# simon-ging/coot-videotext

Measured on AMD Instinct MI355X. Metric: clip-pairs/sec (COOT retrieval train step, whole job), higher is better.
Workload: dtype bf16; 1 GPU; ActivityNet-shaped paper config (anet_coot): 64 videos x 4 clips per GPU, Lc=Lv=80, Ls=16, Lp=64, Dv=2048, Dt=1536, d_model=384; global_batch_videos=64, parallelism=dp1, mode=train, launch=native, deterministic=True, batches=two different synthetic batches in turn

## Files before the change

### coot-videotext_amd/csrc/api.hip

```cpp
#include <stdarg.h>
#include <stdio.h>
#include <string.h>

#include <algorithm>
#include <mutex>
#include <string>
#include <unordered_map>
#include <vector>

#include "../../include/coot_hip.h"
#include "attention.h"
#include "common.h"
#include "fused.h"
#include "gemm.h"
#include "loss.h"
#include "pool.h"
#include "ref_f32.h"
#include "rowops.h"

namespace coot {

static thread_local char g_err[512] = "";
static thread_local hipStream_t g_glob_flush_stream = nullptr;
static thread_local hipEvent_t g_glob_flush_ev = nullptr;
// ... 568 lines not shown
using namespace coot;

extern "C" {

const char* coot_last_error(void) { return coot::g_err; }
int coot_version(void) { return COOT_ABI_VERSION; }
int coot_debug_dropout_scales(uint64_t seed, unsigned site, uint64_t idx0, int64_t n, float p, float* out_host) {
  COOT_REQUIRE(out_host && n >= 0 && p > 0.f, "debug_dropout_scales: bad arguments");
  const DropCfg d = mkdrop(1, p, seed, site);
  const unsigned key = drop_key(seed, site);
  for (int64_t i = 0; i < n; ++i) out_host[i] = drop_scale_key(key, idx0 + (uint64_t)i, d.thr, d.inv_keep);
  return 0;
}
int coot_debug_attn_dropout_scales(uint64_t seed, unsigned site, unsigned row32, int Lk, float p, float* out_host) {
  COOT_REQUIRE(out_host && Lk >= 0 && p > 0.f, "debug_attn_dropout_scales: bad arguments");
  const DropCfg d = mkdrop(1, p, seed, site);
  const unsigned key = drop_key(seed, site);
  for (int k = 0; k < Lk; ++k) out_host[k] = attn_drop_scale(key, row32, k, (unsigned)(Lk + 1) >> 1, d.thr, d.inv_keep);
  return 0;
}
int coot_debug_timestamps(void* dev_u64) { g_fz_tstamps = (unsigned long long*)dev_u64; return 0; }
extern "C" void coot_step_stamps_enable(int on);
extern "C" void coot_step_grad_write(int on);
extern "C" int coot_internal_stage_hits(void);
extern "C" int coot_internal_stream_counter(int which);
extern "C++" { namespace coot { int det_bypass_count(); } }
int coot_get_option(const char* name, int* value) {
  if (!value) { set_error("get_option: null result"); return -1; }
  if (!strcmp(name, "tn_dma")) { *value = get_tn_dma(); return 0; }
  if (!strcmp(name, "xcd_order")) { *value = get_xcd_order(); return 0; }
  if (!strcmp(name, "tn_mode")) { *value = get_tn_mode(); return 0; }
  if (!strcmp(name, "stage_hits")) { *value = coot_internal_stage_hits(); return 0; }
  if (!strcmp(name, "fused_attn_launches")) { *value = fused_attn_launches(); return 0; }
  if (!strcmp(name, "stream_overlap_tests")) { *value = coot_internal_stream_counter(0); return 0; }
  if (!strcmp(name, "stream_candidates_rejected")) { *value = coot_internal_stream_counter(1); return 0; }
  if (!strcmp(name, "stream_unresolved")) { *value = coot_internal_stream_counter(2); return 0; }
  if (!strcmp(name, "operand_f16")) { *value = COOT_OPERAND_IS_F16; return 0; }
  if (!strcmp(name, "det_bypasses")) { *value = det_bypass_count(); return 0; }
  set_error("get_option: unknown or write-only option %s", name);
  return -2;
}
int coot_set_option(const char* name, int value) {
  if (!strcmp(name, "tn_mode")) { set_tn_mode(value); return 0; }
  if (!strcmp(name, "step_stamps")) { coot_step_stamps_enable(value); return 0; }
  if (!strcmp(name, "fused")) { g_use_fused = value; return 0; }
  if (!strcmp(name, "glob_fused")) { g_use_glob_fused = value; return 0; }
  if (!strcmp(name, "glob_fused_bwd")) { g_use_glob_fused_bwd = value; return 0; }
  if (!strcmp(name, "packed")) { g_use_packed = value; return 0; }
  if (!strcmp(name, "fused_infc")) { g_use_fused_infc = value; return 0; }
  if (!strcmp(name, "fused_attn")) { set_fused_attn(value); return 0; }
  if (!strcmp(name, "tn_dma")) { set_tn_dma(value); return 0; }
  if (!strcmp(name, "pack_lazy")) { g_pack_lazy = value; return 0; }
  if (!strcmp(name, "pack_poison")) { g_pack_poison = value; return 0; }
  if (!strcmp(name, "grad_poison")) { g_grad_poison = value; return 0; }
  if (!strcmp(name, "tn_target_wgs")) { set_tn_target_wgs(value); return 0; }
  if (!strcmp(name, "xcd_order")) { set_xcd_order(value); return 0; }
  if (!strcmp(name, "grad_write")) { coot_step_grad_write(value); return 0; }
  if (!strcmp(name, "glob_flush_aux")) { g_glob_flush_aux = value; return 0; }
  if (!strcmp(name, "pool_handover")) { g_pool_handover_on = value; return 0; }
  if (!strcmp(name, "cl_col_split")) { set_cl_col_split(value); return 0; }
  if (!strcmp(name, "cl_small")) { set_cl_small(value); return 0; }
  if (!strcmp(name, "fz_debug")) { g_fz_debug = value; return 0; }
  if (!strcmp(name, "fused_min_rows")) { g_fused_min_rows = value; return 0; }
  set_error("unknown option %s", name);
  return -2;
}

int64_t coot_net_param_numel(const coot_net_config* cfg) {
  coot_net_config c; if (norm_cfg(cfg, &c)) return -1;
  NetLayout L; build_layout(c, L); return L.total;
}
int coot_net_param_count(const coot_net_config* cfg) {
  coot_net_config c; if (norm_cfg(cfg, &c)) return -1;
  NetLayout L; build_layout(c, L); return (int)L.entries.size();
}
int coot_net_param_info(const coot_net_config* cfg, int index, char* name, int name_len, int64_t* offset, int64_t shape[4], int* ndim) {
  coot_net_config c; RUN(norm_cfg(cfg, &c));
  NetLayout L; build_layout(c, L);
  COOT_REQUIRE(index >= 0 && index < (int)L.entries.size(), "param index %d out of range", index);
  const PEntry& e = L.entries[index];
// ... 155 lines not shown
  const coot_net_config* cfgs[1] = {cfg}; const float* Ps[1] = {P}; void* ws[1] = {wpack};
  return coot_nets_pack_weights(1, cfgs, Ps, ws, stream);
}

size_t coot_net_saved_bytes(const coot_net_config* cfg, int N, int Lseq, int N2, int L2) {
  coot_net_config c; if (norm_cfg(cfg, &c)) return 0;
  if (c.dtype == COOT_DTYPE_F32) {
    NetLayout L; build_layout(c, L);
    return ref_f32_workspace_bytes(ref_desc(c, L, N + N2), (long)N * Lseq + (long)N2 * L2);
  }
  Arena A(nullptr, 0); Saved S; layout_saved(c, N + N2, (long)N * Lseq + (long)N2 * L2, A, S); return A.off + 256;
}
size_t coot_net_scratch_bytes(const coot_net_config* cfg, int N, int Lseq, int N2, int L2) {
  coot_net_config c; if (norm_cfg(cfg, &c)) return 0;
  if (c.dtype == COOT_DTYPE_F32) {
    NetLayout L; build_layout(c, L);
    return ref_f32_scratch_bytes(ref_desc(c, L, N + N2), (long)N * Lseq + (long)N2 * L2);
  }
  Arena A(nullptr, 0); Scratch S; layout_scratch(c, N + N2, (long)N * Lseq + (long)N2 * L2, A, S); return A.off + 256;
}

static thread_local int g_grad_overwrite = 0;
int coot_net_grads_overwrite(int on) { g_grad_overwrite = on ? 1 : 0; return 0; }

struct ZeroRanges { float* p[64]; int n[64]; int poison[64]; int count; };
__global__ __launch_bounds__(256) void zero_ranges_kernel(ZeroRanges r) {
  float* p = r.p[blockIdx.x];
  const int n = r.n[blockIdx.x];
  const float v = r.poison[blockIdx.x] ? __uint_as_float(0x7FC00000u) : 0.f;
  for (int i = blockIdx.y * 256 + threadIdx.x; i < n; i += gridDim.y * 256) p[i] = v;
}
static void written_matrices(const coot_net_config& c, const NetLayout& L, std::vector<std::pair<int64_t, int64_t>>& mats) {
  const int64_t D = c.hidden_dim, F = c.ff_dim, Din = c.input_dim;
  if (c.use_input_fc) mats.push_back({L.in_w, D * Din});
  auto layer = [&](const LayerP& lp) { mats.push_back({lp.wqkv, 3 * D * D}); mats.push_back({lp.wo, D * D}); mats.push_back({lp.w1, F * D}); mats.push_back({lp.w2, D * F}); };
  for (const LayerP& lp : L.layers) layer(lp);
  for (const LayerP& lp : L.ctx) layer(lp);
  if (c.pooler == 0) { mats.push_back({L.pw1, D * (int64_t)c.pool_hidden}); mats.push_back({L.pw2, (int64_t)c.pool_hidden * (D / c.pool_heads)}); }
  std::sort(mats.begin(), mats.end());
}
int coot_debug_written_matrices(const coot_net_config* cfg, int64_t* offsets, int64_t* sizes, int max_ranges) {
  coot_net_config c; if (norm_cfg(cfg, &c)) return -1;
  NetLayout L; build_layout(c, L);
  std::vector<std::pair<int64_t, int64_t>> mats; written_matrices(c, L, mats);
  if ((int)mats.size() > max_ranges) return -1;
  for (size_t i = 0; i < mats.size(); ++i) { offsets[i] = mats[i].first; sizes[i] = mats[i].second; }
  return (int)mats.size();
}
int coot_nets_zero_grads(int nnets, const coot_net_config* const* cfgs, float* const* grads, int skip_matrices, coot_stream_t stream) {
  return coot_nets_zero_grads_ex(nnets, cfgs, grads, skip_matrices, nullptr, nullptr, 0, stream);
}
int coot_nets_zero_grads_ex(int nnets, const coot_net_config* const* cfgs, float* const* grads, int skip_matrices, float* const* extra,
                            const int64_t* extra_n, int n_extra, coot_stream_t stream) {
  hipStream_t st = (hipStream_t)stream;
  COOT_REQUIRE(nnets >= 1 && nnets <= 8 && cfgs && grads && (n_extra == 0 || (extra && extra_n)), "nets_zero_grads: bad arguments");
  ZeroRanges zr; zr.count = 0;
  auto flush = [&]() -> int {
    if (zr.count == 0) return 0;
    int big = 0;
    for (int i = 0; i < zr.count; ++i) if (zr.n[i] > big) big = zr.n[i];
    const int gy = big > (1 << 16) ? 64 : 2;
    hipLaunchKernelGGL(zero_ranges_kernel, dim3(zr.count, gy), dim3(256), 0, st, zr);
    COOT_CHECK_LAUNCH("zero_ranges");
    zr.count = 0;
    return 0;
  };
  auto add = [&](float* p, int64_t n, int poison) -> int {
    if (n <= 0) return 0;
    if (zr.count == 64) RUN(flush());
    zr.p[zr.count] = p; zr.n[zr.count] = (int)n; zr.poison[zr.count] = poison; ++zr.count;
    return 0;
  };
  for (int k = 0; k < nnets; ++k) {
    coot_net_config c; RUN(norm_cfg(cfgs[k], &c));
    NetLayout L; build_layout(c, L);
    if (!skip_matrices) { RUN(check_hip(hipMemsetAsync(grads[k], 0, (size_t)L.total * sizeof(float), st), "memset grads")); continue; }
    std::vector<std::pair<int64_t, int64_t>> mats; written_matrices(c, L, mats);
    int64_t pos = 0;
    for (const auto& m : mats) {
      COOT_REQUIRE(m.first >= pos && m.first + m.second <= L.total, "nets_zero_grads: parameter layout");
      RUN(add(grads[k] + pos, m.first - pos, 0));
      if (g_grad_poison) RUN(add(grads[k] + m.first, m.second, 1));
      pos = m.first + m.second;
    }
    RUN(add(grads[k] + pos, L.total - pos, 0));
  }
  for (int e = 0; e < n_extra; ++e)
    for (int64_t o = 0; o < extra_n[e]; o += (1 << 30)) RUN(add(extra[e] + o, extra_n[e] - o < (1 << 30) ? extra_n[e] - o : (1 << 30), 0));
  return flush();
}

struct InputStage { bf16_t* xhat = nullptr; int* pos = nullptr; int mode = 0; };
thread_local InputStage g_input_stage;
void coot_internal_set_input_stage(void* xhat, void* pos, int mode) {
  g_input_stage.xhat = (bf16_t*)xhat; g_input_stage.pos = (int*)pos; g_input_stage.mode = mode;
}

int coot_net_fwd(const coot_net_config* cfg, const float* P, const void* wpack, const float* pe, const float* feats,
                 const int64_t* lengths, int N, int Lseq, const float* feats2, const int64_t* lengths2, int N2, int L2,
                 const float* hidden, float* pooled, float* per_token, void* saved,
                 size_t saved_bytes, void* scratch, size_t scratch_bytes, int train, uint64_t seed, const uint64_t* seed_dev,
                 coot_stream_t stream, const coot_packed_seqs* packed) {
  hipStream_t st = (hipStream_t)stream;
  struct SeedScope { SeedScope(const uint64_t* p) { g_seed_dev = (const unsigned long long*)p; } ~SeedScope() { g_seed_dev = nullptr; } } seedscope(seed_dev);
  coot_net_config c; RUN(norm_cfg(cfg, &c));
  COOT_REQUIRE(P && wpack && pe && feats && lengths && pooled && saved, "net_fwd: null pointer");
  if (packed && packed->source != COOT_SOURCE_PADDED && N2 > 0 && !feats2) feats2 = feats;
  COOT_REQUIRE(!c.use_context || hidden, "net_fwd: context network needs hidden state (transformer_legacy.py:252)");
// ... 339 lines not shown
```

### coot-videotext_amd/csrc/api_step.hip

```cpp
#include <string.h>

#include "../../include/coot_hip.h"
#include "common.h"
#include "det.h"
#include "gemm.h"
#include "fused.h"
#include "pool.h"
#include "rowops.h"

#include <vector>
using namespace coot;

#define RUN(x) do { int _rc = (x); if (_rc) return _rc; } while (0)

namespace {

struct Bump {
  char* base; size_t cap; size_t off = 0; bool overflow = false;
  Bump(void* b, size_t c) : base((char*)b), cap(c) {}
  void* get(size_t bytes) {
    off = (off + 255) & ~(size_t)255;
    char* p = base ? base + off : nullptr;
    off += bytes;
    if (base && off > cap) overflow = true;
// ... 74 lines not shown
    made = true; return 0;
  }
  int hop(int slot, hipStream_t from, hipStream_t to) {
    if (from == to) return 0;
    RUN(record(slot, from));
    return wait(slot, to);
  }
  int record(int slot, hipStream_t from) {
    RUN(init());
    return check_hip(hipEventRecord(ev[slot], from), "eventRecord");
  }
  int wait(int slot, hipStream_t to) { return check_hip(hipStreamWaitEvent(to, ev[slot], 0), "streamWait"); }
};
thread_local Hops g_hops;
thread_local const uint64_t* g_step_seed_dev = nullptr;
thread_local int g_resh_wait_slot = -1;
thread_local void* g_glob_done[2] = {nullptr, nullptr};

constexpr long kEarlyMinTokens = 8192;
struct EarlyUpdate { bool on[2] = {false, false}; const coot_step_config* cfg = nullptr; const coot_step_buffers* b = nullptr; int64_t step = 0; bool repack = false; };
thread_local EarlyUpdate g_early;
int early_update_fire(int side, int gi, hipStream_t st);
int g_grad_write = 1;
int pack_nets(const coot_step_config& c, const coot_step_buffers& b, const int* nets, int count, void* stream) {
  const coot_net_config* cfgs[4]; const float* Ps[4]; void* ws[4];
  for (int k = 0; k < count; ++k) { cfgs[k] = &c.net[nets[k]]; Ps[k] = b.params[nets[k]]; ws[k] = b.wpack[nets[k]]; }
  return coot_nets_pack_weights(count, cfgs, Ps, ws, stream);
}

struct StepStamps {
  static constexpr int MAXN = 40;
  hipEvent_t ev[MAXN]; const char* label[MAXN]; int n = 0, made = 0; bool on = false;
  void begin() { n = 0; }
  void mark(const char* what, hipStream_t st) {
    if (!on || n >= MAXN) return;
    if (made <= n) { if (hipEventCreate(&ev[n]) != hipSuccess) return; made = n + 1; }
    if (hipEventRecord(ev[n], st) != hipSuccess) return;
    label[n++] = what;
  }
};
StepStamps g_stamps;

extern "C" void coot_internal_set_input_stage(void* xhat, void* pos, int mode);
extern "C" void coot_internal_set_glob_flush_stream(void* stream);
extern "C" void coot_internal_set_pool_pack(const long long* counts, int B, int Cmax, float* out, unsigned char* mask, long long* lens);
extern "C" int coot_internal_pool_handover_taken(void);
// ... 174 lines not shown
  glob_xcd_set(li == 0 ? 0 : 4, 4);
  const int rc_gf = coot_net_fwd(&c.net[gi], b.params[gi], b.wpack[gi], b.pe[gi], resh, item_num, d.B, Cmax, nullptr, nullptr, 0, 0,
                                 local_out , glob_out, nullptr, saved_g, sz_g, nullptr, 0, train, seed + 11 * gi,
                                 g_step_seed_dev, st, nullptr);
  glob_xcd_set(0, 8);
  RUN(rc_gf);
  g_stamps.mark(li == 0 ? "video: global forward done" : "text: global forward done", st);
  return 0;
}

int side_backward(const coot_step_config& c, const coot_step_buffers& b, int li, int gi, const float* ctx_feat, const int64_t* ctx_len,
                  int Lctx, const float* item_feat, const int64_t* item_len, int Litem, const int64_t* item_num, int Cmax,
                  const coot_step_dims& d, const float* local_out, const float* resh, float* d_local, const float* d_glob,
                  const float* d_resh, float* dhid, float* dfeat, void* saved_l, size_t sz_l, void* saved_g, size_t sz_g, void* scratch,
                  size_t sz_scratch, int train, uint64_t seed, hipStream_t st, const coot_packed_seqs* pk = nullptr) {
  const int D = c.net[0].hidden_dim;
  g_stamps.mark(li == 0 ? "video: backward starts" : "text: backward starts", st);
  const int side = li == 0 ? 0 : 1;
  const size_t sz_loc = align256(coot_net_scratch_bytes(&c.net[li], d.B, Lctx, d.Nc, Litem));
  const size_t sz_glob = coot_net_scratch_bytes(&c.net[gi], d.B, Cmax, 0, 0);
  COOT_REQUIRE(sz_loc + sz_glob <= sz_scratch, "step backward: scratch too small (%zu < %zu)", sz_scratch, sz_loc + sz_glob);
  glob_xcd_set(side == 0 ? 0 : 4, 4);
  if (g_early.on[side] && g_pipe.init() == 0) coot_internal_set_glob_flush_stream(g_pipe.stream);
  const int rc_g = coot_net_bwd(&c.net[gi], b.params[gi], b.wpack[gi], b.pe[gi], resh, item_num, d.B, Cmax, nullptr, nullptr, 0, 0, local_out, d_glob,
                                b.grads[gi], dhid, dfeat, saved_g, sz_g, (char*)scratch + sz_loc, sz_glob, train, seed + 11 * gi, g_step_seed_dev, st,
                                nullptr);
  glob_xcd_set(0, 8);
  coot_internal_set_glob_flush_stream(nullptr);
  RUN(rc_g);
  g_stamps.mark(li == 0 ? "video: global backward done" : "text: global backward done", st);
  if (g_glob_done[side]) {
    if (det_on()) RUN(det_flush_range(b.grads[gi], (size_t)coot_net_param_numel(&c.net[gi]) * sizeof(float), st));
    RUN(check_hip(hipEventRecord((hipEvent_t)g_glob_done[side], st), "eventRecord"));
  }
  if (g_early.on[side]) RUN(early_update_fire(side, gi, st));
  if (g_resh_wait_slot >= 0 && li == 0) RUN(g_hops.wait(g_resh_wait_slot, st));
  RUN(launch_pack_bwd_join(dfeat, d_resh, dhid, (const long long*)item_num, d.B, Cmax, D, d_local + (size_t)d.B * D, d_local, st));
  const int rc = coot_net_bwd(&c.net[li], b.params[li], b.wpack[li], b.pe[li], ctx_feat, ctx_len, d.B, Lctx, item_feat, item_len, d.Nc, Litem,
                              nullptr, d_local, b.grads[li], nullptr, nullptr, saved_l, sz_l, scratch, sz_loc, train, seed + 11 * li, g_step_seed_dev,
                              st, pk);
  RUN(rc);
  if (det_on()) {
    RUN(det_flush_range(b.grads[li], (size_t)coot_net_param_numel(&c.net[li]) * sizeof(float), st));
    RUN(det_flush_range(b.grads[gi], (size_t)coot_net_param_numel(&c.net[gi]) * sizeof(float), st));
  }
  g_stamps.mark(li == 0 ? "video: local backward done" : "text: local backward done", st);
  return 0;
}

__global__ void sample_idx_kernel(const long long* lens_a, const long long* lens_b, int B, unsigned long long seed, long long* idx,
                                  const unsigned long long* seed_dev = nullptr) {
  const int i = blockIdx.x * blockDim.x + threadIdx.x;
  if (i >= 2 * B) return;
  seed = eff_seed(seed, seed_dev);
  const long long len = i < B ? lens_a[i] : lens_b[i - B];
  const unsigned r = rng_u32(seed, 0xCCu, (unsigned long long)i);
  long long v = (long long)(((unsigned long long)r * (unsigned long long)len) >> 32);
  idx[i] = v < len ? v : len - 1;
}

struct OptK { int mode; float lr, b1, b2, eps, wd, a, b; };

__device__ __forceinline__ void opt_update(const OptK& k, float& p, float g, float& m, float& v, float d) {
  if (k.mode == 0) {
    const float gj = g + k.wd * d * p;
// ... 11 lines not shown
      p -= k.a * k.lr * m;
    }
  }
}

__device__ __forceinline__ void opt_update_range(const OptK& k, float* p, const float* g, float* m, float* v, const float* decay, long i, long n) {
  if (i + 3 < n) {
    f32x4_t pp = *reinterpret_cast<f32x4_t*>(p + i), gg = *reinterpret_cast<const f32x4_t*>(g + i);
    f32x4_t mm = *reinterpret_cast<f32x4_t*>(m + i), vv = *reinterpret_cast<f32x4_t*>(v + i);
    f32x4_t dd = decay ? *reinterpret_cast<const f32x4_t*>(decay + i) : f32x4_t{1.f, 1.f, 1.f, 1.f};
#pragma unroll
    for (int j = 0; j < 4; ++j) { float pj = pp[j], mj = mm[j], vj = vv[j]; opt_update(k, pj, gg[j], mj, vj, dd[j]); pp[j] = pj; mm[j] = mj; vv[j] = vj; }
    if (k.mode != 3) *reinterpret_cast<f32x4_t*>(p + i) = pp;
    *reinterpret_cast<f32x4_t*>(m + i) = mm; *reinterpret_cast<f32x4_t*>(v + i) = vv;
  } else {
    for (long e = i; e < n; ++e) opt_update(k, p[e], g[e], m[e], v[e], decay ? decay[e] : 1.f);
  }
}

__global__ __launch_bounds__(256) void adam_kernel(float* p, const float* g, float* m, float* v, const float* decay, long n, OptK k) {
  for (long i = ((long)blockIdx.x * 256 + threadIdx.x) * 4; i < n; i += (long)gridDim.x * 1024) opt_update_range(k, p, g, m, v, decay, i, n);
}

struct AdamSegs { float* p[4]; const float* g[4]; float* m[4]; float* v[4]; const float* decay[4]; const unsigned char* all1[4]; long n[4]; int blk0[5]; float* losses; };
__global__ __launch_bounds__(256) void adam4_kernel(AdamSegs sg, OptK k_arg, const OptK* k_dev) {
  const OptK k = k_dev ? *k_dev : k_arg;
  int s = 0;
#pragma unroll
  for (int t = 1; t < 4; ++t) if ((int)blockIdx.x >= sg.blk0[t]) s = t;
  if (sg.losses && blockIdx.x == 0 && threadIdx.x == 0) sg.losses[0] = sg.losses[1] + sg.losses[2];
  const long n = sg.n[s];
  const int blk = (int)blockIdx.x - sg.blk0[s];
  const long i = ((long)blk * 256 + threadIdx.x) * 4;
  if (i >= n) return;
  const float* decay = (sg.all1[s] && sg.all1[s][blk]) ? nullptr : sg.decay[s];
  opt_update_range(k, sg.p[s], sg.g[s], sg.m[s], sg.v[s], decay, i, n);
}

__host__ __device__ OptK opt_scalars(int optimizer, int radam_degentosgd, float lr, float beta1, float beta2, float eps, float wd, int64_t step) {
  OptK k; k.lr = lr; k.b1 = beta1; k.b2 = beta2; k.eps = eps; k.wd = wd; k.a = 0.f; k.b = 0.f;
  const double b1t = pow((double)beta1, (double)step), b2t = pow((double)beta2, (double)step);
  if (optimizer == 0) {
    k.mode = 0; k.a = (float)(1.0 / (1.0 - b1t)); k.b = (float)(1.0 / sqrt(1.0 - b2t));
  } else {
    const double nmax = 2.0 / (1.0 - (double)beta2) - 1.0;
    const double nsma = nmax - 2.0 * (double)step * b2t / (1.0 - b2t);
    if (nsma >= 5.0) {
      k.mode = 1;
      k.a = (float)(sqrt((1.0 - b2t) * (nsma - 4.0) / (nmax - 4.0) * (nsma - 2.0) / nsma * nmax / (nmax - 2.0)) / (1.0 - b1t));
    } else if (radam_degentosgd) {
      k.mode = 2; k.a = (float)(1.0 / (1.0 - b1t));
    } else {
      k.mode = 3;
    }
  }
  return k;
}

__global__ void loss_total_kernel(float* losses) { losses[0] = losses[1] + losses[2]; }

struct StepState { unsigned long long seed, step; float lr; int pad; OptK k; };
thread_local StepState* g_state_dev = nullptr;
__global__ void step_state_kernel(StepState* s, int optimizer, int degen, float b1, float b2, float eps, float wd, unsigned long long seed_inc) {
  s->step += 1; s->seed += seed_inc;
  s->k = opt_scalars(optimizer, degen, s->lr, b1, b2, eps, wd, (int64_t)s->step);
}

int adam_nets(const coot_step_config& cfg, const coot_step_buffers& b, const int* nets, int count, int64_t step, hipStream_t st,
              float* losses = nullptr) {
  AdamSegs sg;
  sg.losses = losses;
  int blk = 0;
  for (int k = 0; k < 4; ++k) {
    const int i = nets[k < count ? k : count - 1];
    const long n = k < count ? (long)coot_net_param_numel(&cfg.net[i]) : 0;
    sg.p[k] = b.params[i]; sg.g[k] = b.grads[i]; sg.m[k] = b.adam_m[i]; sg.v[k] = b.adam_v[i]; sg.decay[k] = b.decay_mask[i]; sg.n[k] = n;
    sg.all1[k] = b.decay_mask[i] ? b.decay_block_all[i] : nullptr;
    sg.blk0[k] = blk;
    blk += (int)((n / 4 + 255) / 256);
  }
  sg.blk0[4] = blk;
  const OptK k = opt_scalars(cfg.optimizer, cfg.radam_degentosgd, cfg.lr, cfg.beta1, cfg.beta2, cfg.eps, cfg.weight_decay, step);
  hipLaunchKernelGGL(adam4_kernel, dim3(blk), dim3(256), 0, st, sg, k, g_state_dev ? (const OptK*)&g_state_dev->k : (const OptK*)nullptr);
  COOT_CHECK_LAUNCH("adam4");
  return 0;
}

thread_local const int64_t* g_cc_idx_inject = nullptr;
int draw_cycle_indices(const coot_step_batch& x, const coot_step_dims& d, uint64_t seed, long long* idx, hipStream_t s) {
  if (g_cc_idx_inject)
    return check_hip(hipMemcpyAsync(idx, g_cc_idx_inject, 2 * (size_t)d.B * sizeof(long long), hipMemcpyDeviceToDevice, s), "cycle indices");
  hipLaunchKernelGGL(sample_idx_kernel, dim3((2 * d.B + 255) / 256), dim3(256), 0, s, (const long long*)x.clip_num, (const long long*)x.sent_num,
                     d.B, (unsigned long long)seed, idx, (const unsigned long long*)g_step_seed_dev);
  COOT_CHECK_LAUNCH("sample_idx");
  return 0;
}

int early_update_fire(int side, int gi, hipStream_t st) {
  RUN(g_pipe.init());
  RUN(g_hops.hop(11 + side, st, g_pipe.stream));
  const int nets[1] = {gi};
  RUN(adam_nets(*g_early.cfg, *g_early.b, nets, 1, g_early.step, g_pipe.stream));
  if (g_early.repack) RUN(pack_nets(*g_early.cfg, *g_early.b, nets, 1, g_pipe.stream));
  return g_hops.record(13 + side, g_pipe.stream);
}

}

extern "C" {

static int optimizer_step(int optimizer, int degen, float* params, const float* grads, float* m, float* v, const float* decay_mask, int64_t n,
                          float lr, float beta1, float beta2, float eps, float weight_decay, int64_t step, coot_stream_t stream) {
  COOT_REQUIRE(params && grads && m && v && step >= 1, "optimizer step: bad arguments");
  if (n <= 0) return 0;
  int blocks = (int)((n / 4 + 255) / 256);
  if (blocks > 2048) blocks = 2048;
  if (blocks < 1) blocks = 1;
  hipLaunchKernelGGL(adam_kernel, dim3(blocks), dim3(256), 0, (hipStream_t)stream, params, grads, m, v, decay_mask, (long)n,
                     opt_scalars(optimizer, degen, lr, beta1, beta2, eps, weight_decay, step));
  COOT_CHECK_LAUNCH("optimizer step");
  return 0;
}

int coot_adam_step(float* params, const float* grads, float* m, float* v, const float* decay_mask, int64_t n, float lr, float beta1,
                   float beta2, float eps, float weight_decay, int64_t step, coot_stream_t stream) {
// ... 169 lines not shown
  if (cc) {
    RUN(draw_cycle_indices(*x, *d, seed, W.idx, st));
    RUN(coot_cyclecons_fwd_bwd(W.resh_v, W.resh_t, x->clip_num, x->sent_num, (const int64_t*)W.idx, (const int64_t*)(W.idx + d->B), d->B,
                               d->Cmax_clip, d->Cmax_sent, D, cfg->cc_weight, 1.0f / (float)d->B, losses + 2, nullptr, nullptr, W.d_resh_v,
                               W.d_resh_t, side_t));
    g_stamps.mark("text: cycle-consistency done", st);
  }
  RUN(coot_contrastive_fwd_bwd_part(&cfg->contr, d->B, d->Nc, 2 * D, D, W.glob_v, W.glob_t, W.local_v + (size_t)d->B * D,
                                    W.local_t + (size_t)d->B * D, W.local_v, W.local_t, losses + 1, W.d_glob_v, W.d_glob_t,
                                    W.d_local_v + (size_t)d->B * D, W.d_local_t + (size_t)d->B * D, W.d_local_v, W.d_local_t, W.loss_scratch,
                                    W.sz_loss, COOT_CONTRASTIVE_LOCAL, side_t));
  g_stamps.mark("text: local contrastive terms done", st);
  RUN(g_hops.record(7, st));
  RUN(g_hops.wait(2, sv));
  g_stamps.mark("video: text forward joined", sv);
  RUN(coot_contrastive_fwd_bwd_part(&cfg->contr, d->B, d->Nc, 2 * D, D, W.glob_v, W.glob_t, W.local_v + (size_t)d->B * D,
                                    W.local_t + (size_t)d->B * D, W.local_v, W.local_t, losses + 1, W.d_glob_v, W.d_glob_t,
                                    W.d_local_v + (size_t)d->B * D, W.d_local_t + (size_t)d->B * D, W.d_local_v, W.d_local_t, W.loss_scratch,
                                    W.sz_loss, COOT_CONTRASTIVE_GLOBAL, side_v));
  g_stamps.mark("video: contrastive done", sv);
  RUN(g_hops.hop(3, sv, st));
  const int vnets[2] = {0, 1}, tnets[2] = {2, 3};
  g_resh_wait_slot = 7;
  const bool early = optimize && !det_on() && !g_state_dev;
  const bool early_v = early && (long)d->B * d->Lv + (long)d->Nc * d->Lc >= kEarlyMinTokens;
  const bool early_t = early && (long)d->B * d->Lp + (long)d->Nc * d->Ls >= kEarlyMinTokens;
  struct EarlyScope { ~EarlyScope() { g_early = EarlyUpdate{}; } } early_scope;
  g_early.on[0] = early_v; g_early.on[1] = early_t; g_early.cfg = cfg; g_early.b = b; g_early.step = step; g_early.repack = repack;
  (void)coot_net_grads_overwrite(g_grad_write);
  if (piped) coot_internal_set_input_stage(SL.xv, SL.pv, 0);
  const int rc_v = side_backward(*cfg, *b, 0, 1, x->vid_feat, x->vid_len, d->Lv, x->clip_feat, x->clip_len, d->Lc, x->clip_num, d->Cmax_clip, *d,
                                 W.local_v, W.resh_v, W.d_local_v, W.d_glob_v, cc ? W.d_resh_v : nullptr, W.dhid_v, W.dfeat_v, W.saved_lv, W.sz_lv,
                                 W.saved_gv, W.sz_gv, W.scratch_v, W.sz_sv, train, seed, sv, &pk.v);
  g_resh_wait_slot = -1;
  if (rc_v) (void)coot_net_grads_overwrite(0);
  RUN(rc_v);
  if (det_on()) RUN(det_flush_range(losses, 3 * sizeof(float), sv));
  if (optimize) RUN(adam_nets(*cfg, *b, vnets, early_v ? 1 : 2, step, sv, losses));
  else {
    hipLaunchKernelGGL(loss_total_kernel, dim3(1), dim3(1), 0, sv, losses);
    COOT_CHECK_LAUNCH("loss_total");
  }
  if (repack) RUN(pack_nets(*cfg, *b, vnets, early_v ? 1 : 2, side_v));
  if (early_v) RUN(g_hops.wait(13, sv));
  g_stamps.mark("video: updated", sv);
  if (piped) coot_internal_set_input_stage(SL.xt, SL.pt, 0);
  const int rc_t = side_backward(*cfg, *b, 2, 3, x->par_feat, x->par_len, d->Lp, x->sent_feat, x->sent_len, d->Ls, x->sent_num, d->Cmax_sent, *d, W.local_t,
                                 W.resh_t, W.d_local_t, W.d_glob_t, cc ? W.d_resh_t : nullptr, W.dhid_t, W.dfeat_t, W.saved_lt, W.sz_lt, W.saved_gt, W.sz_gt,
                                 W.scratch_t, W.sz_st, train, seed + 1000, st, &pk.t);
  (void)coot_net_grads_overwrite(0);
  coot_internal_set_input_stage(nullptr, nullptr, 0);
  RUN(rc_t);
  if (optimize) RUN(adam_nets(*cfg, *b, tnets, early_t ? 1 : 2, step, st));
  if (repack) RUN(pack_nets(*cfg, *b, tnets, early_t ? 1 : 2, side_t));
  if (early_t) RUN(g_hops.wait(14, st));
  g_stamps.mark("text: updated", st);
  RUN(g_hops.hop(4, sv, sm));
  if ((do_optimizer & COOT_STEP_DEFER_TEXT_JOIN) == 0) RUN(g_hops.hop(5, st, sm));
  g_stamps.mark("step done", sm);
  return 0;
}

void coot_step_stamps_enable(int on) { g_stamps.on = on != 0; }
int coot_internal_stage_hits(void) { return g_pipe.hits; }
size_t coot_step_device_state_bytes(void) { return sizeof(StepState); }
int coot_step_set_device_state(void* state) {
  g_state_dev = (StepState*)state;
  g_step_seed_dev = state ? (const uint64_t*)&g_state_dev->seed : nullptr;
  return 0;
}
int coot_step_set_cycle_indices(const int64_t* idx) { g_cc_idx_inject = idx; return 0; }
size_t coot_step_input_stage_bytes(const coot_step_config* cfg, const coot_step_dims* dims) {
  if (!cfg || !dims) return 0;
  return stage_layout(*cfg, *dims, nullptr).bytes;
}
int coot_step_set_input_stages(void* stage0, void* stage1, size_t bytes_each) {
// ... 50 lines not shown
  COOT_REQUIRE(out && n_others >= 0 && n_others <= 8 && (others || n_others == 0), "stream_create_concurrent: arguments");
  hipStream_t must[8];
  for (int i = 0; i < n_others; ++i) must[i] = (hipStream_t)others[i];
  hipStream_t s = nullptr;
  const hipStream_t nice[1] = {g_pipe.stream};
  RUN(g_streams.create(must, n_others, nice, g_pipe.stream ? 1 : 0, priority, &s, concurrent));
  g_streams.live.push_back(s);
  *out = (coot_stream_t)s;
  return 0;
}
int coot_stream_destroy(coot_stream_t s) {
  for (size_t i = 0; i < g_streams.live.size(); ++i)
    if (g_streams.live[i] == (hipStream_t)s) {
      g_streams.live.erase(g_streams.live.begin() + i);
      RUN(check_hip(hipStreamSynchronize((hipStream_t)s), "streamSynchronize"));
      if (g_pipe.checked && (g_pipe.beside[0] == (hipStream_t)s || g_pipe.beside[1] == (hipStream_t)s)) g_pipe.checked = false;
      return check_hip(hipStreamDestroy((hipStream_t)s), "streamDestroy");
    }
  set_error("stream_destroy: not a stream of coot_stream_create_concurrent (of this thread)");
  return 1;
}
int coot_internal_stream_counter(int which) { return which == 0 ? g_streams.tests : (which == 1 ? g_streams.rejected : g_streams.unresolved); }
void coot_step_grad_write(int on) { g_grad_write = on ? 1 : 0; }

int coot_debug_step_stamps(char* buf, int buf_bytes) {
  if (!buf || buf_bytes <= 0) return 0;
  buf[0] = 0;
  if (g_stamps.n == 0) return 0;
  if (hipDeviceSynchronize() != hipSuccess) return -1;
  int off = 0;
  for (int i = 0; i < g_stamps.n; ++i) {
    float ms = 0.f;
    if (hipEventElapsedTime(&ms, g_stamps.ev[0], g_stamps.ev[i]) != hipSuccess) ms = -1.f;
    off += snprintf(buf + off, off < buf_bytes ? buf_bytes - off : 0, "%9.1f us  %s\n", ms * 1e3f, g_stamps.label[i]);
    if (off >= buf_bytes) break;
  }
  return g_stamps.n;
}

}
```

### coot-videotext_amd/csrc/det.h

```cpp
#pragma once
#include "common.h"

namespace coot {

struct DetRange { const char* base; size_t bytes; long long* shadow; };
struct DetTable { int n; DetRange r[8]; unsigned* bypass; };
constexpr double kDetScale = 1099511627776.0;
constexpr float kDetMaxAddend = 4194304.0f;

static __device__ DetTable g_det_dev = {0, {}, nullptr};

__device__ __forceinline__ void acc_add(float* p, float v) {
  const int n = g_det_dev.n;
  for (int i = 0; i < n; ++i) {
    const size_t off = (size_t)(reinterpret_cast<const char*>(p) - g_det_dev.r[i].base);
    if (off < g_det_dev.r[i].bytes) {
      if (!(fabsf(v) < kDetMaxAddend)) {
        atomicAdd(g_det_dev.bypass, 1u);
        break;
      }
      atomicAdd(reinterpret_cast<unsigned long long*>(g_det_dev.r[i].shadow + (off >> 2)), (unsigned long long)llrint((double)v * kDetScale));
      return;
    }
  }
  atomicAdd(p, v);
}

#define COOT_DET_DEFINE_SETTER(name)                                                                              \
  int det_set_table_##name(const DetTable& t) {                                                                   \
    return check_hip(hipMemcpyToSymbol(HIP_SYMBOL(g_det_dev), &t, sizeof(DetTable)), "det table (" #name ")");   \
  }

int det_set_table_fused(const DetTable& t);
int det_set_table_gemm(const DetTable& t);
int det_set_table_loss(const DetTable& t);
int det_set_table_pool(const DetTable& t);
int det_set_table_rowops(const DetTable& t);
int det_flush_range(const void* base, size_t bytes, hipStream_t st);
bool det_on();
int det_bypass_count();

}
```

### coot-videotext_amd/csrc/det.hip

```cpp
#include "det.h"

#include "../../include/coot_hip.h"

namespace coot {
namespace {
DetTable g_host_table = {0, {}, nullptr};

__global__ __launch_bounds__(256) void det_flush_kernel(float* p, long long* shadow, long n) {
  for (long i = (long)blockIdx.x * 256 + threadIdx.x; i < n; i += (long)gridDim.x * 256) {
    const long long v = shadow[i];
    if (v != 0) {
      shadow[i] = 0;
      p[i] += (float)((double)v * (1.0 / kDetScale));
    }
  }
}
}

bool det_on() { return g_host_table.n > 0; }

int det_bypass_count() {
  if (g_host_table.n <= 0 || !g_host_table.bypass) return -1;
  unsigned v = 0;
  if (check_hip(hipDeviceSynchronize(), "det bypass count") || check_hip(hipMemcpy(&v, g_host_table.bypass, 4, hipMemcpyDeviceToHost), "det bypass count")) return -1;
  return (int)(v > 0x7fffffffu ? 0x7fffffffu : v);
}

int det_flush_range(const void* base, size_t bytes, hipStream_t st) {
  const char* b0 = (const char*)base;
  for (int i = 0; i < g_host_table.n; ++i) {
    const DetRange& R = g_host_table.r[i];
    const char* lo = b0 > R.base ? b0 : R.base;
    const char* hi = (b0 + bytes) < (R.base + R.bytes) ? (b0 + bytes) : (R.base + R.bytes);
    if (lo >= hi) continue;
    const long n = (hi - lo) / 4, first = (lo - R.base) / 4;
    int blocks = (int)((n + 1023) / 1024);
    if (blocks > 1024) blocks = 1024;
    if (blocks < 1) blocks = 1;
    hipLaunchKernelGGL(det_flush_kernel, dim3(blocks), dim3(256), 0, st, (float*)const_cast<char*>(lo), R.shadow + first, n);
// ... 46 lines not shown
```

### coot-videotext_amd/csrc/gemm.hip

```cpp
#include "gemm.h"
#include "det.h"
#include <algorithm>
#include "rowops.h"

namespace coot {

constexpr int BN = 128;
constexpr int BK = 64;
constexpr int PITCH = BK + 16;
constexpr int CPITCH = BN + 4;

__device__ __forceinline__ u32x4_t load16_guard(const bf16_t* p, bool ok) {
  u32x4_t z = {0u, 0u, 0u, 0u};
  if (ok) z = *reinterpret_cast<const u32x4_t*>(p);
  return z;
}

__device__ __forceinline__ void unpack8(u32x4_t u, float* v) {
  v[0] = bflo(u[0]); v[1] = bfhi(u[0]); v[2] = bflo(u[1]); v[3] = bfhi(u[1]);
  v[4] = bflo(u[2]); v[5] = bfhi(u[2]); v[6] = bflo(u[3]); v[7] = bfhi(u[3]);
}
__device__ __forceinline__ u32x4_t pack8(const float* v) {
  return u32x4_t{pack2bf(v[0], v[1]), pack2bf(v[2], v[3]), pack2bf(v[4], v[5]), pack2bf(v[6], v[7])};
}
// ... 1261 lines not shown
  if (g_tn_collect && !g.ws) {
    if (g_tn_nitems == TN_MAX_ITEMS) { int rc = tn_batch_flush(stream); if (rc) return rc; }
    g_tn_items[g_tn_nitems++] = g;
    return 0;
  }
  if (g.overwrite) {
    COOT_REQUIRE(g.groups == 1 && g.ldc == g.No, "gemm_tn: overwrite needs a dense single-group C");
    int rc = launch_fill_f32(g.C, (long)g.Mo * g.No, 0.f, stream);
    if (rc) return rc;
    GemmTN g2 = g; g2.overwrite = 0;
    return launch_gemm_tn(g2, stream);
  }
  int splits = tn_splits(g.T, g.Mo, g.No, g.groups);
  int t_per_split = (g.T + splits - 1) / splits;
  t_per_split = (t_per_split + TN_BT - 1) / TN_BT * TN_BT;
  splits = (g.T + t_per_split - 1) / t_per_split;
  float* ws = nullptr;
  const size_t need = (size_t)splits * g.groups * g.Mo * g.No;
  if (g.ws && need <= g.ws_floats) ws = g.ws;
  else if (!g.ws && g_tn_ws && need <= g_tn_ws_floats) ws = g_tn_ws;
  dim3 grid((g.No + TN_BC - 1) / TN_BC, (g.Mo + TN_BC - 1) / TN_BC, g.groups * splits);
  const int direct = (splits == 1 && g.ldc % 4 == 0 && g.No % 4 == 0 && g.zC % 4 == 0) ? 1 : 0;
  if (direct) ws = nullptr;
  void* ts = timing_begin(TIMING_TN, 2.0 * g.T * g.Mo * g.No * g.groups, 0, stream);
  if (g_tn_mode == 0)
    hipLaunchKernelGGL(gemm_tn_kernel<0>, grid, dim3(256), 0, stream, g, t_per_split, splits, ws, direct);
  else
    hipLaunchKernelGGL(gemm_tn_kernel<1>, grid, dim3(256), 0, stream, g, t_per_split, splits, ws, direct);
  COOT_CHECK_LAUNCH("gemm_tn");
  if (ws) {
    const long total4 = (long)g.Mo * g.No * g.groups / 4;
    int blocks = (int)((total4 + 255) / 256);
    if (blocks > 1024) blocks = 1024;
    hipLaunchKernelGGL(gemm_tn_reduce_kernel, dim3(blocks), dim3(256), 0, stream, g, splits, ws);
    COOT_CHECK_LAUNCH("gemm_tn_reduce");
  }
  timing_end(ts, stream);
  return 0;
}

}

namespace coot {
COOT_DET_DEFINE_SETTER(gemm)
}
```

Baseline: 207,700 clip-pairs/s.

## Fold deterministic shadow flush into Adam and restrict flush to accumulated gradient segments

In deterministic mode the whole gradient arena was flushed from its fixed-point shadow after each backward pass, and this blocked the early per-net optimizer update. The new code flushes only the gradient ranges that are actually accumulated atomically, and it folds that flush (plus the losses) into the Adam kernel itself. This re-enables early updates when deterministic mode is on. The cost is more per-block segment checks inside the Adam kernel and bookkeeping to detect split-K GEMMs that accumulate atomically.

```diff
diff --git a/coot-videotext_amd/csrc/api.hip b/coot-videotext_amd/csrc/api.hip
--- a/coot-videotext_amd/csrc/api.hip
+++ b/coot-videotext_amd/csrc/api.hip
@@ -614,6 +614,8 @@
 int coot_debug_timestamps(void* dev_u64) { g_fz_tstamps = (unsigned long long*)dev_u64; return 0; }
 extern "C" void coot_step_stamps_enable(int on);
 extern "C" void coot_step_grad_write(int on);
+extern "C" void coot_step_det_seg_flush(int on);
+extern "C" int coot_step_det_seg_flush_get(void);
 extern "C" int coot_internal_stage_hits(void);
 extern "C" int coot_internal_stream_counter(int which);
 extern "C++" { namespace coot { int det_bypass_count(); } }
@@ -628,6 +630,7 @@
   if (!strcmp(name, "stream_candidates_rejected")) { *value = coot_internal_stream_counter(1); return 0; }
   if (!strcmp(name, "stream_unresolved")) { *value = coot_internal_stream_counter(2); return 0; }
   if (!strcmp(name, "operand_f16")) { *value = COOT_OPERAND_IS_F16; return 0; }
+  if (!strcmp(name, "det_seg_flush")) { *value = coot_step_det_seg_flush_get(); return 0; }
   if (!strcmp(name, "det_bypasses")) { *value = det_bypass_count(); return 0; }
   set_error("get_option: unknown or write-only option %s", name);
   return -2;
@@ -648,6 +651,7 @@
   if (!strcmp(name, "tn_target_wgs")) { set_tn_target_wgs(value); return 0; }
   if (!strcmp(name, "xcd_order")) { set_xcd_order(value); return 0; }
   if (!strcmp(name, "grad_write")) { coot_step_grad_write(value); return 0; }
+  if (!strcmp(name, "det_seg_flush")) { coot_step_det_seg_flush(value); return 0; }
   if (!strcmp(name, "glob_flush_aux")) { g_glob_flush_aux = value; return 0; }
   if (!strcmp(name, "pool_handover")) { g_pool_handover_on = value; return 0; }
   if (!strcmp(name, "cl_col_split")) { set_cl_col_split(value); return 0; }
@@ -849,6 +853,7 @@
 
 static thread_local int g_grad_overwrite = 0;
 int coot_net_grads_overwrite(int on) { g_grad_overwrite = on ? 1 : 0; return 0; }
+extern "C" int coot_internal_grads_overwrite(void) { return g_grad_overwrite; }
 
 struct ZeroRanges { float* p[64]; int n[64]; int poison[64]; int count; };
 __global__ __launch_bounds__(256) void zero_ranges_kernel(ZeroRanges r) {
@@ -865,6 +870,27 @@
   for (const LayerP& lp : L.ctx) layer(lp);
   if (c.pooler == 0) { mats.push_back({L.pw1, D * (int64_t)c.pool_hidden}); mats.push_back({L.pw2, (int64_t)c.pool_hidden * (D / c.pool_heads)}); }
   std::sort(mats.begin(), mats.end());
+}
+static int accumulated_ranges(const coot_net_config& c, const NetLayout& L, std::vector<std::pair<int64_t, int64_t>>& acc,
+                              std::vector<std::pair<int64_t, int64_t>>* mats_out = nullptr) {
+  std::vector<std::pair<int64_t, int64_t>> mats; written_matrices(c, L, mats);
+  int64_t pos = 0;
+  for (const auto& m : mats) {
+    COOT_REQUIRE(m.first >= pos && m.first + m.second <= L.total, "gradient arena: parameter layout");
+    if (m.first > pos) acc.push_back({pos, m.first - pos});
+    pos = m.first + m.second;
+  }
+  if (L.total > pos) acc.push_back({pos, L.total - pos});
+  if (mats_out) *mats_out = mats;
+  return 0;
+}
+extern "C" int coot_internal_grad_accum_ranges(const coot_net_config* cfg, int64_t* offsets, int64_t* sizes, int max_ranges) {
+  coot_net_config c; RUN(norm_cfg(cfg, &c));
+  NetLayout L; build_layout(c, L);
+  std::vector<std::pair<int64_t, int64_t>> acc; RUN(accumulated_ranges(c, L, acc));
+  COOT_REQUIRE((int)acc.size() <= max_ranges, "grad_accum_ranges: %d ranges (room for %d)", (int)acc.size(), max_ranges);
+  for (size_t i = 0; i < acc.size(); ++i) { offsets[i] = acc[i].first; sizes[i] = acc[i].second; }
+  return (int)acc.size();
 }
 int coot_debug_written_matrices(const coot_net_config* cfg, int64_t* offsets, int64_t* sizes, int max_ranges) {
   coot_net_config c; if (norm_cfg(cfg, &c)) return -1;
@@ -902,15 +928,10 @@
     coot_net_config c; RUN(norm_cfg(cfgs[k], &c));
     NetLayout L; build_layout(c, L);
     if (!skip_matrices) { RUN(check_hip(hipMemsetAsync(grads[k], 0, (size_t)L.total * sizeof(float), st), "memset grads")); continue; }
-    std::vector<std::pair<int64_t, int64_t>> mats; written_matrices(c, L, mats);
-    int64_t pos = 0;
-    for (const auto& m : mats) {
-      COOT_REQUIRE(m.first >= pos && m.first + m.second <= L.total, "nets_zero_grads: parameter layout");
-      RUN(add(grads[k] + pos, m.first - pos, 0));
-      if (g_grad_poison) RUN(add(grads[k] + m.first, m.second, 1));
-      pos = m.first + m.second;
-    }
-    RUN(add(grads[k] + pos, L.total - pos, 0));
+    std::vector<std::pair<int64_t, int64_t>> acc, mats; RUN(accumulated_ranges(c, L, acc, &mats));
+    for (const auto& a : acc) RUN(add(grads[k] + a.first, a.second, 0));
+    if (g_grad_poison)
+      for (const auto& m : mats) RUN(add(grads[k] + m.first, m.second, 1));
   }
   for (int e = 0; e < n_extra; ++e)
     for (int64_t o = 0; o < extra_n[e]; o += (1 << 30)) RUN(add(extra[e] + o, extra_n[e] - o < (1 << 30) ? extra_n[e] - o : (1 << 30), 0));
diff --git a/coot-videotext_amd/csrc/api_step.hip b/coot-videotext_amd/csrc/api_step.hip
--- a/coot-videotext_amd/csrc/api_step.hip
+++ b/coot-videotext_amd/csrc/api_step.hip
@@ -120,6 +120,26 @@
 thread_local EarlyUpdate g_early;
 int early_update_fire(int side, int gi, hipStream_t st);
 int g_grad_write = 1;
+
+extern "C" int coot_internal_grad_accum_ranges(const coot_net_config* cfg, int64_t* offsets, int64_t* sizes, int max_ranges);
+extern "C" int coot_internal_grads_overwrite(void);
+int g_det_seg = 1;
+struct DetPlan {
+  bool fold = false;
+  bool full[4] = {true, true, true, true};
+  float* losses = nullptr;
+};
+thread_local DetPlan g_det_plan;
+int det_arena_segs(const coot_step_config& c, const coot_step_buffers& b, int net, DetSegs& out, hipStream_t st) {
+  const long n = (long)coot_net_param_numel(&c.net[net]);
+  if (g_det_plan.full[net]) return det_segs_add(out, b.grads[net], n, st);
+  int64_t off[64], len[64];
+  const int k = coot_internal_grad_accum_ranges(&c.net[net], off, len, 64);
+  if (k < 0) return k;
+  for (int i = 0; i < k; ++i) RUN(det_segs_add(out, b.grads[net] + off[i], (long)len[i], st));
+  return 0;
+}
+void det_plan_arena(int net) { g_det_plan.full[net] = !coot_internal_grads_overwrite() || det_take_matrix_atomics(); }
 int pack_nets(const coot_step_config& c, const coot_step_buffers& b, const int* nets, int count, void* stream) {
   const coot_net_config* cfgs[4]; const float* Ps[4]; void* ws[4];
   for (int k = 0; k < count; ++k) { cfgs[k] = &c.net[nets[k]]; Ps[k] = b.params[nets[k]]; ws[k] = b.wpack[nets[k]]; }
@@ -340,25 +360,42 @@
   COOT_REQUIRE(sz_loc + sz_glob <= sz_scratch, "step backward: scratch too small (%zu < %zu)", sz_scratch, sz_loc + sz_glob);
   glob_xcd_set(side == 0 ? 0 : 4, 4);
   if (g_early.on[side] && g_pipe.init() == 0) coot_internal_set_glob_flush_stream(g_pipe.stream);
+  (void)det_take_matrix_atomics();
   const int rc_g = coot_net_bwd(&c.net[gi], b.params[gi], b.wpack[gi], b.pe[gi], resh, item_num, d.B, Cmax, nullptr, nullptr, 0, 0, local_out, d_glob,
                                 b.grads[gi], dhid, dfeat, saved_g, sz_g, (char*)scratch + sz_loc, sz_glob, train, seed + 11 * gi, g_step_seed_dev, st,
                                 nullptr);
   glob_xcd_set(0, 8);
   coot_internal_set_glob_flush_stream(nullptr);
   RUN(rc_g);
+  det_plan_arena(gi);
   g_stamps.mark(li == 0 ? "video: global backward done" : "text: global backward done", st);
+  const bool seg = det_on() && g_det_seg;
   if (g_glob_done[side]) {
-    if (det_on()) RUN(det_flush_range(b.grads[gi], (size_t)coot_net_param_numel(&c.net[gi]) * sizeof(float), st));
+    if (seg) {
+      DetSegs ds;
+      RUN(det_arena_segs(c, b, gi, ds, st));
+      RUN(det_flush_segs(ds, st));
+    } else if (det_on()) {
+      RUN(det_flush_range(b.grads[gi], (size_t)coot_net_param_numel(&c.net[gi]) * sizeof(float), st));
+    }
     RUN(check_hip(hipEventRecord((hipEvent_t)g_glob_done[side], st), "eventRecord"));
   }
   if (g_early.on[side]) RUN(early_update_fire(side, gi, st));
   if (g_resh_wait_slot >= 0 && li == 0) RUN(g_hops.wait(g_resh_wait_slot, st));
   RUN(launch_pack_bwd_join(dfeat, d_resh, dhid, (const long long*)item_num, d.B, Cmax, D, d_local + (size_t)d.B * D, d_local, st));
+  (void)det_take_matrix_atomics();
   const int rc = coot_net_bwd(&c.net[li], b.params[li], b.wpack[li], b.pe[li], ctx_feat, ctx_len, d.B, Lctx, item_feat, item_len, d.Nc, Litem,
                               nullptr, d_local, b.grads[li], nullptr, nullptr, saved_l, sz_l, scratch, sz_loc, train, seed + 11 * li, g_step_seed_dev,
                               st, pk);
   RUN(rc);
-  if (det_on()) {
+  det_plan_arena(li);
+  if (seg && !g_det_plan.fold) {
+    DetSegs ds;
+    RUN(det_arena_segs(c, b, li, ds, st));
+    if (!g_glob_done[side]) RUN(det_arena_segs(c, b, gi, ds, st));
+    if (side == 0 && g_det_plan.losses) RUN(det_segs_add(ds, g_det_plan.losses, 3, st));
+    RUN(det_flush_segs(ds, st));
+  } else if (det_on() && !seg) {
     RUN(det_flush_range(b.grads[li], (size_t)coot_net_param_numel(&c.net[li]) * sizeof(float), st));
     RUN(det_flush_range(b.grads[gi], (size_t)coot_net_param_numel(&c.net[gi]) * sizeof(float), st));
   }
@@ -416,17 +453,43 @@
   for (long i = ((long)blockIdx.x * 256 + threadIdx.x) * 4; i < n; i += (long)gridDim.x * 1024) opt_update_range(k, p, g, m, v, decay, i, n);
 }
 
-struct AdamSegs { float* p[4]; const float* g[4]; float* m[4]; float* v[4]; const float* decay[4]; const unsigned char* all1[4]; long n[4]; int blk0[5]; float* losses; };
+constexpr int kAdamFlushSegs = 64;
+struct AdamSegs {
+  float* p[4]; float* g[4]; float* m[4]; float* v[4]; const float* decay[4]; const unsigned char* all1[4]; long n[4]; int blk0[5]; float* losses;
+  long long* sh[4]; long long* loss_sh; int fseg0[5]; int flo[kAdamFlushSegs], fhi[kAdamFlushSegs];
+};
 __global__ __launch_bounds__(256) void adam4_kernel(AdamSegs sg, OptK k_arg, const OptK* k_dev) {
   const OptK k = k_dev ? *k_dev : k_arg;
   int s = 0;
 #pragma unroll
   for (int t = 1; t < 4; ++t) if ((int)blockIdx.x >= sg.blk0[t]) s = t;
-  if (sg.losses && blockIdx.x == 0 && threadIdx.x == 0) sg.losses[0] = sg.losses[1] + sg.losses[2];
+  if (sg.losses && blockIdx.x == 0 && threadIdx.x == 0) {
+    if (sg.loss_sh)
+      for (int w = 0; w < 3; ++w) {
+        const long long v = sg.loss_sh[w];
+        if (v != 0) { sg.loss_sh[w] = 0; sg.losses[w] = det_fold(sg.losses[w], v); }
+      }
+    sg.losses[0] = sg.losses[1] + sg.losses[2];
+  }
   const long n = sg.n[s];
   const int blk = (int)blockIdx.x - sg.blk0[s];
   const long i = ((long)blk * 256 + threadIdx.x) * 4;
   if (i >= n) return;
+  if (long long* sh = sg.sh[s]) {
+    const long b0 = (long)blk * 1024, b1 = b0 + 1024;
+    float* g = sg.g[s];
+    for (int q = sg.fseg0[s]; q < sg.fseg0[s + 1]; ++q) {
+      const long lo = sg.flo[q], hi = sg.fhi[q];
+      if (lo >= b1 || hi <= b0) continue;
+#pragma unroll
+      for (int j = 0; j < 4; ++j) {
+        const long e = i + j;
+        if (e < lo || e >= hi || e >= n) continue;
+        const long long v = sh[e];
+        if (v != 0) { sh[e] = 0; g[e] = det_fold(g[e], v); }
+      }
+    }
+  }
   const float* decay = (sg.all1[s] && sg.all1[s][blk]) ? nullptr : sg.decay[s];
   opt_update_range(k, sg.p[s], sg.g[s], sg.m[s], sg.v[s], decay, i, n);
 }
@@ -461,10 +524,17 @@
 }
 
 int adam_nets(const coot_step_config& cfg, const coot_step_buffers& b, const int* nets, int count, int64_t step, hipStream_t st,
-              float* losses = nullptr) {
+              float* losses = nullptr, bool flush = false) {
   AdamSegs sg;
   sg.losses = losses;
-  int blk = 0;
+  sg.loss_sh = nullptr;
+  flush = flush && det_on();
+  DetSegs spill;
+  if (flush && losses) {
+    const int where = det_locate(losses, 3 * sizeof(float), &sg.loss_sh);
+    if (where < 0) RUN(det_segs_add(spill, losses, 3, st));
+  }
+  int blk = 0, nseg = 0;
   for (int k = 0; k < 4; ++k) {
     const int i = nets[k < count ? k : count - 1];
     const long n = k < count ? (long)coot_net_param_numel(&cfg.net[i]) : 0;
@@ -472,8 +542,24 @@
     sg.all1[k] = b.decay_mask[i] ? b.decay_block_all[i] : nullptr;
     sg.blk0[k] = blk;
     blk += (int)((n / 4 + 255) / 256);
-  }
-  sg.blk0[4] = blk;
+    sg.sh[k] = nullptr; sg.fseg0[k] = nseg;
+    if (!flush || k >= count) continue;
+    DetSegs ds;
+    RUN(det_arena_segs(cfg, b, i, ds, st));
+    if (ds.n == 0) continue;
+    bool fits = nseg + ds.n <= kAdamFlushSegs && n <= (1L << 30);
+    for (int q = 0; q < ds.n && fits; ++q) fits = ds.s[q].shadow - (ds.s[q].p - b.grads[i]) == ds.s[0].shadow - (ds.s[0].p - b.grads[i]);
+    if (!fits) {
+      for (int q = 0; q < ds.n; ++q) RUN(det_segs_add(spill, ds.s[q].p, ds.s[q].n, st));
+      continue;
+    }
+    sg.sh[k] = ds.s[0].shadow - (ds.s[0].p - b.grads[i]);
+    for (int q = 0; q < ds.n; ++q) {
+      sg.flo[nseg] = (int)(ds.s[q].p - b.grads[i]); sg.fhi[nseg] = sg.flo[nseg] + ds.s[q].n; ++nseg;
+    }
+  }
+  sg.blk0[4] = blk; sg.fseg0[4] = nseg;
+  RUN(det_flush_segs(spill, st));
   const OptK k = opt_scalars(cfg.optimizer, cfg.radam_degentosgd, cfg.lr, cfg.beta1, cfg.beta2, cfg.eps, cfg.weight_decay, step);
   hipLaunchKernelGGL(adam4_kernel, dim3(blk), dim3(256), 0, st, sg, k, g_state_dev ? (const OptK*)&g_state_dev->k : (const OptK*)nullptr);
   COOT_CHECK_LAUNCH("adam4");
@@ -494,7 +580,7 @@
   RUN(g_pipe.init());
   RUN(g_hops.hop(11 + side, st, g_pipe.stream));
   const int nets[1] = {gi};
-  RUN(adam_nets(*g_early.cfg, *g_early.b, nets, 1, g_early.step, g_pipe.stream));
+  RUN(adam_nets(*g_early.cfg, *g_early.b, nets, 1, g_early.step, g_pipe.stream, nullptr, g_det_plan.fold));
   if (g_early.repack) RUN(pack_nets(*g_early.cfg, *g_early.b, nets, 1, g_pipe.stream));
   return g_hops.record(13 + side, g_pipe.stream);
 }
@@ -710,7 +796,9 @@
   RUN(g_hops.hop(3, sv, st));
   const int vnets[2] = {0, 1}, tnets[2] = {2, 3};
   g_resh_wait_slot = 7;
-  const bool early = optimize && !det_on() && !g_state_dev;
+  struct DetScope { ~DetScope() { g_det_plan = DetPlan{}; } } det_scope;
+  g_det_plan.fold = optimize && g_det_seg; g_det_plan.losses = losses;
+  const bool early = optimize && (!det_on() || g_det_seg) && !g_state_dev;
   const bool early_v = early && (long)d->B * d->Lv + (long)d->Nc * d->Lc >= kEarlyMinTokens;
   const bool early_t = early && (long)d->B * d->Lp + (long)d->Nc * d->Ls >= kEarlyMinTokens;
   struct EarlyScope { ~EarlyScope() { g_early = EarlyUpdate{}; } } early_scope;
@@ -723,8 +811,8 @@
   g_resh_wait_slot = -1;
   if (rc_v) (void)coot_net_grads_overwrite(0);
   RUN(rc_v);
-  if (det_on()) RUN(det_flush_range(losses, 3 * sizeof(float), sv));
-  if (optimize) RUN(adam_nets(*cfg, *b, vnets, early_v ? 1 : 2, step, sv, losses));
+  if (det_on() && !g_det_seg) RUN(det_flush_range(losses, 3 * sizeof(float), sv));
+  if (optimize) RUN(adam_nets(*cfg, *b, vnets, early_v ? 1 : 2, step, sv, losses, g_det_plan.fold));
   else {
     hipLaunchKernelGGL(loss_total_kernel, dim3(1), dim3(1), 0, sv, losses);
     COOT_CHECK_LAUNCH("loss_total");
@@ -739,7 +827,7 @@
   (void)coot_net_grads_overwrite(0);
   coot_internal_set_input_stage(nullptr, nullptr, 0);
   RUN(rc_t);
-  if (optimize) RUN(adam_nets(*cfg, *b, tnets, early_t ? 1 : 2, step, st));
+  if (optimize) RUN(adam_nets(*cfg, *b, tnets, early_t ? 1 : 2, step, st, nullptr, g_det_plan.fold));
   if (repack) RUN(pack_nets(*cfg, *b, tnets, early_t ? 1 : 2, side_t));
   if (early_t) RUN(g_hops.wait(14, st));
   g_stamps.mark("text: updated", st);
@@ -836,6 +924,8 @@
 }
 int coot_internal_stream_counter(int which) { return which == 0 ? g_streams.tests : (which == 1 ? g_streams.rejected : g_streams.unresolved); }
 void coot_step_grad_write(int on) { g_grad_write = on ? 1 : 0; }
+void coot_step_det_seg_flush(int on) { g_det_seg = on ? 1 : 0; }
+int coot_step_det_seg_flush_get(void) { return g_det_seg; }
 
 int coot_debug_step_stamps(char* buf, int buf_bytes) {
   if (!buf || buf_bytes <= 0) return 0;
diff --git a/coot-videotext_amd/csrc/det.h b/coot-videotext_amd/csrc/det.h
--- a/coot-videotext_amd/csrc/det.h
+++ b/coot-videotext_amd/csrc/det.h
@@ -37,6 +37,17 @@
 int det_set_table_pool(const DetTable& t);
 int det_set_table_rowops(const DetTable& t);
 int det_flush_range(const void* base, size_t bytes, hipStream_t st);
+
+__device__ __forceinline__ float det_fold(float w, long long v) { return __fadd_rn(w, (float)((double)v * (1.0 / kDetScale))); }
+
+int det_locate(const void* base, size_t bytes, long long** shadow);
+constexpr int kDetMaxSegs = 64;
+struct DetSeg { float* p; long long* shadow; int n; int blk0; };
+struct DetSegs { int n = 0; DetSeg s[kDetMaxSegs]; };
+int det_segs_add(DetSegs& s, float* p, long n, hipStream_t st);
+int det_flush_segs(DetSegs& s, hipStream_t st);
+void det_note_matrix_atomics();
+bool det_take_matrix_atomics();
 bool det_on();
 int det_bypass_count();
 
diff --git a/coot-videotext_amd/csrc/det.hip b/coot-videotext_amd/csrc/det.hip
--- a/coot-videotext_amd/csrc/det.hip
+++ b/coot-videotext_amd/csrc/det.hip
@@ -11,10 +11,64 @@
     const long long v = shadow[i];
     if (v != 0) {
       shadow[i] = 0;
-      p[i] += (float)((double)v * (1.0 / kDetScale));
+      p[i] = det_fold(p[i], v);
     }
   }
 }
+
+__global__ __launch_bounds__(256) void det_flush_segs_kernel(DetSegs sg) {
+  int s = 0;
+  for (int t = 1; t < sg.n; ++t) if ((int)blockIdx.x >= sg.s[t].blk0) s = t;
+  const DetSeg& g = sg.s[s];
+  const int i0 = ((int)blockIdx.x - g.blk0) * 1024 + threadIdx.x;
+#pragma unroll
+  for (int k = 0; k < 4; ++k) {
+    const int i = i0 + k * 256;
+    if (i >= g.n) break;
+    const long long v = g.shadow[i];
+    if (v != 0) {
+      g.shadow[i] = 0;
+      g.p[i] = det_fold(g.p[i], v);
+    }
+  }
+}
+thread_local bool g_matrix_atomics = false;
+}
+
+void det_note_matrix_atomics() { g_matrix_atomics = true; }
+bool det_take_matrix_atomics() { const bool r = g_matrix_atomics; g_matrix_atomics = false; return r; }
+
+int det_locate(const void* base, size_t bytes, long long** shadow) {
+  const char* b0 = (const char*)base;
+  *shadow = nullptr;
+  for (int i = 0; i < g_host_table.n; ++i) {
+    const DetRange& R = g_host_table.r[i];
+    if (b0 >= R.base && b0 + bytes <= R.base + R.bytes) { *shadow = R.shadow + (b0 - R.base) / 4; return 1; }
+    if (b0 < R.base + R.bytes && b0 + bytes > R.base) return -1;
+  }
+  return 0;
+}
+
+int det_segs_add(DetSegs& s, float* p, long n, hipStream_t st) {
+  if (n <= 0 || !det_on()) return 0;
+  long long* sh = nullptr;
+  const int where = det_locate(p, (size_t)n * sizeof(float), &sh);
+  if (where < 0) return det_flush_range(p, (size_t)n * sizeof(float), st);
+  if (where == 0) return 0;
+  COOT_REQUIRE(n <= (1L << 30), "det segments: %ld words", n);
+  if (s.n == kDetMaxSegs) { const int rc = det_flush_segs(s, st); if (rc) return rc; }
+  s.s[s.n++] = DetSeg{p, sh, (int)n, 0};
+  return 0;
+}
+
+int det_flush_segs(DetSegs& s, hipStream_t st) {
+  if (s.n == 0) return 0;
+  int blk = 0;
+  for (int i = 0; i < s.n; ++i) { s.s[i].blk0 = blk; blk += (s.s[i].n + 1023) / 1024; }
+  hipLaunchKernelGGL(det_flush_segs_kernel, dim3(blk), dim3(256), 0, st, s);
+  COOT_CHECK_LAUNCH("det_flush_segs");
+  s.n = 0;
+  return 0;
 }
 
 bool det_on() { return g_host_table.n > 0; }
diff --git a/coot-videotext_amd/csrc/gemm.hip b/coot-videotext_amd/csrc/gemm.hip
--- a/coot-videotext_amd/csrc/gemm.hip
+++ b/coot-videotext_amd/csrc/gemm.hip
@@ -1307,6 +1307,7 @@
   dim3 grid((g.No + TN_BC - 1) / TN_BC, (g.Mo + TN_BC - 1) / TN_BC, g.groups * splits);
   const int direct = (splits == 1 && g.ldc % 4 == 0 && g.No % 4 == 0 && g.zC % 4 == 0) ? 1 : 0;
   if (direct) ws = nullptr;
+  if (!ws && !direct && det_on()) det_note_matrix_atomics();
   void* ts = timing_begin(TIMING_TN, 2.0 * g.T * g.Mo * g.No * g.groups, 0, stream);
   if (g_tn_mode == 0)
     hipLaunchKernelGGL(gemm_tn_kernel<0>, grid, dim3(256), 0, stream, g, t_per_split, splits, ws, direct);
```

Measured after the change: 214,300 clip-pairs/s (median of 6 runs). 3.2% higher.
